# gdoteof/pytorch-zappa-serverless

Hardware: AMD Instinct MI355X
Metric: inferences/sec (whole node) + p50 cold-start ms, ResNet-50 bs=1 at 1/2/4/8 GPU (higher is better)
Workload: dtype bf16

## Files before the change

hipzap/_native.py:

```python
from __future__ import annotations

import ctypes as C
import os
import threading

DEBUG = os.environ.get("HIPZAP_DEBUG") == "1"
_LIB_PATH = os.path.join(os.path.dirname(os.path.realpath(__file__)), "_lib",
                         "libhipzap_debug.so" if DEBUG else "libhipzap.so")
if os.environ.get("HIPZAP_LIB"):
    _LIB_PATH = os.path.realpath(os.environ["HIPZAP_LIB"])
DEBUG_UNITS = ("conv", "gemm", "vision", "transformer", "lstm", "lmbatch", "pack", "block")
_lock = threading.Lock()
_lib = None

c_void_p, c_int, c_long, c_double = C.c_void_p, C.c_int, C.c_long, C.c_double
c_float_p = C.POINTER(C.c_float)

KINDS = {
    "HZ_K_CONV": 1, "HZ_K_LAYERNORM": 2, "HZ_K_EMBED": 3, "HZ_K_ATTENTION": 4, "HZ_K_VIT_TOKENS": 5,
    "HZ_K_LSTM": 6, "HZ_K_DECODER": 7, "HZ_K_SAMPLER": 8, "HZ_K_MAXPOOL": 9, "HZ_K_QUANT": 10,
    "HZ_K_GEMM_FP8": 11, "HZ_K_SOFTMAX": 12, "HZ_K_POOL_FC": 13, "HZ_K_LMB_LAYER": 14, "HZ_K_LMB_DEC": 15,
    "HZ_K_LMB_ADMIT": 16, "HZ_K_STEM": 18, "HZ_K_BNECK": 19, "HZ_K_SEAM": 20, "HZ_K_KCONV": 21,
    "HZ_K_QKVATT": 22, "HZ_K_CONV2": 23, "HZ_K_AVGPOOL": 24, "HZ_K_PREPROCESS": 25, "HZ_K_STEP_BUMP": 26,
    "HZ_K_DIAG": 27, "HZ_K_RESIZE_PREPROCESS": 28,
# ... 196 lines not shown
    _sig(lib, "hz_plan_blob", P, P, C.POINTER(U64))
    _sig(lib, "hz_plan_host", P, P, c_int)
    _sig(lib, "hz_plan_device", P, P, c_int)
    _sig(lib, "hz_plan_stream", P, P, c_int)
    _sig(lib, "hz_plan_upload_stream", P, P)
    _sig(lib, "hz_plan_replay", c_int, P, c_int)
    _sig(lib, "hz_plan_sync", c_int, P, c_int)
    _sig(lib, "hz_plan_infer", c_int, P, c_int, P, U64, U64, P, U64, U64)
    _sig(lib, "hz_plan_bench", D, P, c_int)
    _sig(lib, "hz_plan_close", None, P)
    _sig(lib, "hz_plan_prog", P, P, c_int)
    _sig(lib, "hz_plan_capture_ctx", c_int, P, c_int)
    PP_ = C.POINTER(c_void_p)
    _sig(lib, "hz_exec_create", P, PP_, PP_, PP_, C.POINTER(U64), c_int, PP_, U64, c_int)
    _sig(lib, "hz_exec_create_batched", P, PP_, PP_, PP_, C.POINTER(U64), c_int, PP_, U64, c_int, c_int, D, c_int)
    _sig(lib, "hz_exec_batches", None, P, C.POINTER(U64))
    _sig(lib, "hz_exec_submit", c_int, P, PP_, P, C.POINTER(D))
    _sig(lib, "hz_exec_submit_rows", c_int, P, PP_, c_int, P, C.POINTER(D))
    _sig(lib, "hz_exec_submit_sized", c_int, P, PP_, C.POINTER(U64), P, C.POINTER(D))
    _sig(lib, "hz_exec_stats", None, P, C.POINTER(U64), C.POINTER(U64))
    _sig(lib, "hz_exec_destroy", None, P)
    _sig(lib, "hz_exec_bench", c_int, P, c_int, c_int, PP_, C.POINTER(D), C.POINTER(D))
    _sig(lib, "hz_http_start", P, c_int, P)
    _sig(lib, "hz_http_set_fast", c_int, P, P, c_int, c_int, c_int, c_int, c_int, c_int, C.c_char_p)
    _sig(lib, "hz_http_set_lm", c_int, P, P, c_int, c_int, c_int, c_int, C.c_char_p, U64, C.c_char_p)
    _sig(lib, "hz_http_respond", None, P, c_int, C.c_char_p, U64, C.c_char_p, U64)
    _sig(lib, "hz_http_stats", None, P, C.POINTER(U64))
    _sig(lib, "hz_http_stop", C.c_int, P)
    _sig(lib, "hz_pack_conv_launch", c_int, C.POINTER(PackConvParams), P)
    _sig(lib, "hz_frag_pack_launch", c_int, C.POINTER(FragPackParams), P)
# ... 33 lines not shown
    with _lock:
        if _lib is None:
            if not os.path.exists(_LIB_PATH):
                if os.environ.get("HIPZAP_NO_AUTOBUILD"):
                    raise RuntimeError(f"hipzap native library missing: {_LIB_PATH} (run python -m hipzap.build)")
                from . import build as _b
                _b.build(verbose=False, debug=DEBUG)
            _lib = _load()
    return _lib


def experiments() -> bool:
    return bool(lib().hz_experiments())


def check(rc: int, what: str) -> None:
    if rc != 0:
        raise RuntimeError(f"hipzap native call {what} failed with code {rc}")


def ptr(t) -> int:
    return 0 if t is None else t.data_ptr()


def stream_ptr(stream=None) -> int:
    import torch
    s = stream if stream is not None else torch.cuda.current_stream()
    return s.cuda_stream
```

hipzap/csrc/executor.cpp:

```cpp
#include <hip/hip_runtime.h>

#include <algorithm>
#include <atomic>
#include <chrono>
#include <cstdlib>
#include <condition_variable>
#include <cstring>
#include <deque>
#include <mutex>
#include <thread>
#include <vector>

#include "hipzap.h"

namespace {

constexpr int kMaxIn = 4;

double now_us() {
  return std::chrono::duration<double, std::micro>(std::chrono::steady_clock::now().time_since_epoch()).count();
}

struct Slot {
  HzProgram prog = nullptr;
  hipStream_t st = nullptr;
  void* in[kMaxIn] = {};
  void* out = nullptr;
  hipEvent_t ev = nullptr;
  bool done = false;
  std::atomic<bool> done_a{false};
  int rc = 0;
  std::condition_variable cv;
  int claimed = 0, copied = 0, read = 0;
  bool sealed = false;
  double t_open = 0;
};

struct Exec {
  std::vector<Slot> slots;
  int n_in = 1;
  uint64_t in_bytes[kMaxIn] = {};
  uint64_t out_bytes = 0;
  std::mutex mu;
  std::condition_variable cv_free, cv_work;
  std::vector<int> free_slots;
  std::deque<int> to_launch;
  std::vector<int> inflight;
  bool stop = false;
  int active = 0;
  std::thread worker;
  uint64_t served = 0, polls = 0, batches = 0;
  int rows = 1, open = -1, min_inflight = 1;
  double max_wait_us = 0;
  uint64_t row_in[kMaxIn] = {};
  uint64_t row_out = 0;
  double spin_us = 300.0;
  std::atomic<int> work_hint{0};

  void complete(int s, int rc) {
    std::lock_guard<std::mutex> g(mu);
    slots[s].rc = rc;
    slots[s].done = true;
    slots[s].done_a.store(true, std::memory_order_release);
    slots[s].cv.notify_all();
    served += rows == 1 ? 1 : slots[s].claimed;
    ++batches;
  }

  void queue_if_ready(int s) {
    Slot& sl = slots[s];
    if (sl.sealed && sl.copied == sl.claimed) {
      to_launch.push_back(s);
      work_hint.fetch_add(1, std::memory_order_release);
      cv_work.notify_one();
    }
  }

  void seal_open() {
    const int s = open;
    open = -1;
    slots[s].sealed = true;
    queue_if_ready(s);
  }
// ... 35 lines not shown
      for (size_t i = 0; i < inflight.size();) {
        const int s = inflight[i];
        const hipError_t q = hipEventQuery(slots[s].ev);
        ++polls;
        if (q == hipErrorNotReady) {
          ++i;
          continue;
        }
        complete(s, q == hipSuccess ? 0 : (int)q);
        inflight[i] = inflight.back();
        inflight.pop_back();
        progressed = true;
      }
      if (!progressed) std::this_thread::yield();
    }
  }

  int submit_batched(const void* const* in, void* out, double* lat_us) {
    const double t0 = now_us();
    int s, r;
    {
      std::unique_lock<std::mutex> lk(mu);
      while (open < 0) {
        if (stop) return -10;
        if (!free_slots.empty()) {
          s = free_slots.back();
          free_slots.pop_back();
          Slot& o = slots[s];
          o.claimed = o.copied = o.read = 0;
          o.sealed = o.done = false;
          o.t_open = now_us();
          open = s;
          work_hint.fetch_add(1, std::memory_order_release);
          cv_work.notify_one();
          cv_free.notify_all();
          break;
        }
        cv_free.wait(lk);
      }
      s = open;
      r = slots[s].claimed++;
      if (slots[s].claimed == rows) seal_open();
    }
    Slot& sl = slots[s];
    for (int k = 0; k < n_in; ++k)
      if (in && in[k] && row_in[k]) std::memcpy(static_cast<char*>(sl.in[k]) + r * row_in[k], in[k], row_in[k]);
    int rc;
    {
      std::unique_lock<std::mutex> lk(mu);
      ++sl.copied;
      queue_if_ready(s);
      sl.cv.wait(lk, [&] { return sl.done; });
      rc = sl.rc;
    }
    if (!rc && out && row_out) std::memcpy(out, static_cast<const char*>(sl.out) + r * row_out, row_out);
    {
      std::lock_guard<std::mutex> g(mu);
      if (++sl.read == sl.claimed) {
        free_slots.push_back(s);
        cv_free.notify_all();
      }
// ... 23 lines not shown
            cv_work.notify_one();
            cv_free.notify_all();
            break;
          }
          cv_free.wait(lk);
        }
        s = open;
        r = slots[s].claimed;
        k = std::min(m - done, rows - r);
        slots[s].claimed += k;
        if (slots[s].claimed == rows) seal_open();
      }
      Slot& sl = slots[s];
      for (int q = 0; q < n_in; ++q)
        if (in && in[q] && row_in[q])
          std::memcpy(static_cast<char*>(sl.in[q]) + r * row_in[q], static_cast<const char*>(in[q]) + done * row_in[q],
                      k * row_in[q]);
      {
        std::unique_lock<std::mutex> lk(mu);
        sl.copied += k;
        queue_if_ready(s);
        sl.cv.wait(lk, [&] { return sl.done; });
        rc = sl.rc;
      }
      if (!rc && out && row_out)
        std::memcpy(static_cast<char*>(out) + done * row_out, static_cast<const char*>(sl.out) + r * row_out, k * row_out);
      {
        std::lock_guard<std::mutex> g(mu);
        sl.read += k;
        if (sl.read == sl.claimed) {
          free_slots.push_back(s);
          cv_free.notify_all();
// ... 20 lines not shown
    return rc;
  }

  int submit_one(const void* const* in, void* out, double* lat_us, const uint64_t* nbytes = nullptr) {
    const double t0 = now_us();
    int s;
    {
      std::unique_lock<std::mutex> lk(mu);
      cv_free.wait(lk, [&] { return stop || !free_slots.empty(); });
      if (stop) return -10;
      s = free_slots.back();
      free_slots.pop_back();
    }
    Slot& sl = slots[s];
    for (int k = 0; k < n_in; ++k)
      if (in && in[k] && in_bytes[k]) std::memcpy(sl.in[k], in[k], nbytes ? nbytes[k] : in_bytes[k]);
    int rc;
    bool spin;
    {
      std::unique_lock<std::mutex> lk(mu);
      sl.done = false;
      sl.done_a.store(false, std::memory_order_relaxed);
      to_launch.push_back(s);
      work_hint.fetch_add(1, std::memory_order_release);
      cv_work.notify_one();
      spin = spin_us > 0 && active <= 2;
    }
    if (spin) {
      const double ts = now_us();
      while (!sl.done_a.load(std::memory_order_acquire) && now_us() - ts < 4.0 * spin_us) std::this_thread::yield();
    }
// ... 62 lines not shown
  for (int k = 0; k < n_in; ++k)
    if (in_bytes[k] % rows) return nullptr;
  auto* e = static_cast<Exec*>(hz_exec_create(progs, streams, host_in, in_bytes, n_in, host_out, out_bytes, n));
  if (!e) return nullptr;
  {
    std::lock_guard<std::mutex> g(e->mu);
    e->rows = rows;
    e->max_wait_us = max_wait_us;
    e->min_inflight = min_inflight;
    for (int k = 0; k < n_in; ++k) e->row_in[k] = in_bytes[k] / rows;
    e->row_out = out_bytes / rows;
  }
  return e;
}

void hz_exec_batches(void* h, uint64_t* batches) {
  Exec* e = static_cast<Exec*>(h);
  std::lock_guard<std::mutex> g(e->mu);
  *batches = e->batches;
}

int hz_exec_submit(void* h, const void* const* in, void* out, double* lat_us) {
  return static_cast<Exec*>(h)->submit_wait(in, out, lat_us);
}

int hz_exec_submit_sized(void* h, const void* const* in, const uint64_t* nbytes, void* out, double* lat_us) {
  Exec* e = static_cast<Exec*>(h);
  if (e->rows != 1 || !nbytes) return -1;
  for (int k = 0; k < e->n_in; ++k)
    if (nbytes[k] > e->in_bytes[k]) return -2;
// ... 38 lines not shown
```

hipzap/csrc/hipzap.h:

```cpp
#pragma once
#include <hip/hip_runtime.h>
#include <stdint.h>

#ifdef __cplusplus
extern "C" {
#endif

enum { HZ_ACT_NONE = 0, HZ_ACT_RELU = 1, HZ_ACT_GELU = 2, HZ_ACT_TANH = 3 };

typedef struct HzConvParams {
  const unsigned short* x;
  const unsigned short* w;
  const float* bias;
  const unsigned short* res;
  void* out;
  int N, H, W, C;
  int Cout, R, S, stride, pad, P, Q;
  int M, K, ksteps;
  int act, out_f32, out_rowmajor, ldo;
  int x_rowmajor, ldx;
  int tiles_n;
  int kw;
  const struct HzLnFold* lnf;
  int x_f32;
// ... 458 lines not shown
int hz_prog_add_kernel(HzProgram p, int kind, const void* params, size_t size, int slot);
int hz_prog_add_memcpy(HzProgram p, void* dst, const void* src, size_t bytes, int slot);
int hz_prog_add_fork(HzProgram p, int slot);
int hz_prog_add_join(HzProgram p, int slot);
int hz_prog_run(HzProgram p, hipStream_t st);
int hz_prog_capture(HzProgram p, hipStream_t st);
int hz_prog_replay(HzProgram p, hipStream_t st);
int hz_prog_is_captured(HzProgram p);
int hz_prog_prepare(HzProgram p);
int hz_prog_replay_n(HzProgram p, hipStream_t st, int n);
double hz_prog_bench(HzProgram* progs, hipStream_t* streams, int n, int iters);
int hz_prog_bench2(HzProgram* progs, hipStream_t* streams, int n, int iters, int threads, double* out);
int hz_serve_bench(HzProgram* progs, hipStream_t* streams, void** in_dst, void** in_src, uint64_t in_bytes,
                   void** out_src, void** out_dst, uint64_t out_bytes, int n, int iters, double* lat_us,
                   double* wall_us);
int hz_diag_launch(int kind, int blocks, int threads, void* a, void* b, long bytes, hipStream_t st);

#define HZ_ABI_EPOCH 2
enum { HZ_PLAN_OP_MEMCPY = 6, HZ_PLAN_OP_KERNEL = 7, HZ_PLAN_OP_FORK = 8, HZ_PLAN_OP_JOIN = 9 };
typedef struct HzMemcpyArgs {
  void* dst;
  const void* src;
  uint64_t bytes;
} HzMemcpyArgs;
enum { HZ_PLAN_T_PARSE = 0, HZ_PLAN_T_HIP_INIT = 1, HZ_PLAN_T_UPLOAD = 2, HZ_PLAN_T_CTX_ALLOC = 3,
       HZ_PLAN_T_BIND = 4, HZ_PLAN_T_CAPTURE = 5, HZ_PLAN_T_BLOB_ALLOC = 6,
       HZ_PLAN_T_FIRST_COPY = 7,
       HZ_PLAN_T_STREAM = 8, HZ_PLAN_T_UPLOAD_DMA = 9, HZ_PLAN_T_WARM_WAIT = 10, HZ_PLAN_T_WARM_THREAD = 11,
       HZ_PLAN_NT = 12 };
uint64_t hz_abi_version(void);
// ... 9 lines not shown
void* hz_plan_stream(void* plan, int ctx);
void* hz_plan_upload_stream(void* plan);
int hz_plan_replay(void* plan, int ctx);
int hz_plan_sync(void* plan, int ctx);
int hz_plan_infer(void* plan, int ctx, const void* in, uint64_t in_off, uint64_t in_bytes, void* out,
                  uint64_t out_off, uint64_t out_bytes);
double hz_plan_bench(void* plan, int iters);
HzProgram hz_plan_prog(void* plan, int ctx);
int hz_plan_capture_ctx(void* plan, int ctx);

void* hz_exec_create(HzProgram* progs, hipStream_t* streams, void** host_in, const uint64_t* in_bytes, int n_in,
                     void** host_out, uint64_t out_bytes, int n);
void* hz_exec_create_batched(HzProgram* progs, hipStream_t* streams, void** host_in, const uint64_t* in_bytes,
                             int n_in, void** host_out, uint64_t out_bytes, int n, int rows, double max_wait_us,
                             int min_inflight);
void hz_exec_batches(void* exec, uint64_t* batches);
int hz_exec_submit(void* exec, const void* const* in, void* out, double* lat_us);
int hz_exec_submit_rows(void* exec, const void* const* in, int m, void* out, double* lat_us);
int hz_exec_submit_sized(void* exec, const void* const* in, const uint64_t* nbytes, void* out, double* lat_us);
void hz_exec_stats(void* exec, uint64_t* served, uint64_t* polls);
void hz_exec_destroy(void* exec);
int hz_exec_bench(void* exec, int clients, int iters, const void* const* in, double* lat_us, double* wall_us);

typedef void (*HzHttpPyHandler)(void* req, const char* method, const char* target, const char* headers,
                                uint64_t hlen, const char* body, uint64_t blen);
void* hz_http_start(int listen_fd, HzHttpPyHandler py);
int hz_http_set_fast(void* srv, void* exec, int H, int W, int C, int out_floats, int classes, int probs,
                     const char* model);
int hz_http_set_lm(void* srv, void* sched, int V, int maxn, int dflt, int empty_id, const char* blob, uint64_t blen,
                   const uint8_t* flags);
// ... 9 lines not shown
```

hipzap/csrc/runtime.cpp:

```cpp
#include <hip/hip_runtime.h>
#include <atomic>
#include <chrono>
#include <cstdio>
#include <cstdlib>
#include <cstring>
#include <thread>
#include <vector>

#include "common.h"
#include "hipzap.h"

namespace {

struct Op {
  int slot;
  enum Type { KERNEL, MEMCPY, FORK, JOIN } type;
  int kind;
  std::vector<char> prm;
};

struct Program {
  std::vector<Op> ops;
  std::vector<hipStream_t> side;
  std::vector<hipEvent_t> fork_ev;
  hipGraph_t graph = nullptr;
// ... 199 lines not shown
        if (!rc && out_bytes) memcpy(out_dst[i], out_src[i], out_bytes);
        rcs[i] = rc;
        lat_us[(size_t)i * iters + it] =
            std::chrono::duration<double, std::micro>(std::chrono::steady_clock::now() - a).count();
      }
    });
  for (auto& t : th) t.join();
  *wall_us = std::chrono::duration<double, std::micro>(std::chrono::steady_clock::now() - t0).count();
  int rc = 0;
  for (int r : rcs) rc |= r;
  return rc;
}

}

extern "C" int hz_experiments(void) { return HZ_EXPERIMENTS; }

extern "C" int hz_prog_replay_n(HzProgram h, hipStream_t st, int n) {
  for (int i = 0; i < n; ++i) {
    const int rc = hz_prog_replay(h, st);
    if (rc) return rc;
  }
  return 0;
}

static int hz_conv_op(const HzConvOp* o, hipStream_t st) { return hz_conv_launch(&o->p, o->cfg, st); }
static int hz_conv2_op(const HzConv2Op* o, hipStream_t st) { return hz_conv2_launch(&o->a, &o->b, o->cfg, st); }
static int hz_avgpool_op(const HzAvgpoolArgs* a, hipStream_t st) {
  return hz_avgpool_launch(a->x, a->out, a->N, a->HW, a->C, a->blocked, st);
}
// ... 53 lines not shown
```

hipzap/engine/engine.py:

```python
from __future__ import annotations

import os
import threading
import time

import torch

from .. import _native
from ..models import registry
from .program import ExecContext, bench_contexts, serve_bench_contexts


def load_tuning(model: str, batch: int, contexts: int = 1) -> dict | None:
    import json
    from .tune import table_path
    for c in range(contexts, 0, -1):
        p = table_path(model, batch, c)
        if p.exists():
            with open(p) as f:
                return json.load(f)
    return None


def add_softmax_head(g) -> None:
# ... 153 lines not shown
            return ex
        from ..executor import Executor
        with self._build_lock:
            if getattr(self, "_bexec", None) is not None:
                raise RuntimeError("this engine serves through the dynamic-batching executor")
            if self._exec is None:
                for lk in self._locks:
                    lk.acquire()
                try:
                    cs = self.contexts
                    self._exec = Executor(
                        [c.prog for c in cs], [s.cuda_stream for s in self.streams],
                        [[c.host_inputs[k].data_ptr() for c in cs] for k in range(len(cs[0].host_inputs))],
                        [h.numel() * h.element_size() for h in cs[0].host_inputs],
                        [c.host_output.data_ptr() for c in cs],
                        cs[0].host_output.numel() * cs[0].host_output.element_size())
                finally:
                    for lk in self._locks:
                        lk.release()
        return self._exec

    def infer(self, x) -> torch.Tensor:
        xs = list(x) if isinstance(x, (list, tuple)) else [x]
        ex = self.executor()
        if ex is not None:
            c0 = self.contexts[0]
            hbs = c0.host_inputs
            if all(xi.dtype == hb.dtype and xi.is_contiguous() and xi.numel() == hb.numel() and xi.device.type == "cpu"
                   for hb, xi in zip(hbs, xs)):
                ins = xs
            else:
                ins = [xi.to(hb.dtype).reshape(hb.shape).contiguous() for hb, xi in zip(hbs, xs)]
            out = torch.empty_like(c0.host_output)
            ex.submit([t.data_ptr() for t in ins], out.data_ptr())
            if _native.DEBUG:
                from ..utils import kcheck
                kcheck.check(f"{self.model} infer")
            return self._post(out)
        i = self._pick()
        ctx, s = self.contexts[i], self.streams[i]
        with self._locks[i], torch.cuda.device(self.device), torch.cuda.stream(s):
            if self.host_io:
                for hb, xi in zip(ctx.host_inputs, xs):
                    hb.copy_(xi.reshape(hb.shape))
                ctx.replay(s)
                s.synchronize()
                out = ctx.host_output.clone()
            else:
                for d, xi in zip(ctx.inputs, xs):
                    d.copy_(xi.reshape(d.shape), non_blocking=True)
                ctx.replay(s)
                out = ctx.output.to("cpu", non_blocking=False)
        if _native.DEBUG:
            from ..utils import kcheck
            kcheck.check(f"{self.model} infer")
        return self._post(out)

    @property
    def resize(self) -> dict | None:
# ... 57 lines not shown

    def batched_executor(self, max_wait_us: float = 200.0, min_inflight: int = 1):
        from ..executor import Executor
        self.ensure_contexts()
        with self._build_lock:
            if self._exec is not None:
                raise RuntimeError("this engine already serves through the per-request executor")
            if getattr(self, "_bexec", None) is None:
                cs = self.contexts
                self._bexec = Executor(
                    [c.prog for c in cs], [s.cuda_stream for s in self.streams],
                    [[c.host_inputs[k].data_ptr() for c in cs] for k in range(len(cs[0].host_inputs))],
                    [h.numel() * h.element_size() for h in cs[0].host_inputs],
                    [c.host_output.data_ptr() for c in cs],
                    cs[0].host_output.numel() * cs[0].host_output.element_size(),
                    rows=self.batch, max_wait_us=max_wait_us, min_inflight=min_inflight)
        return self._bexec

    def serve_bench(self, iters: int, payload=None, clients: int | None = None,
                    mode: str = "executor") -> tuple[float, list]:
        self.ensure_contexts()
        c0 = self.contexts[0]
        p = payload if payload is not None else c0.host_input
        p = p.to(c0.host_input.dtype).reshape(c0.host_input.shape).contiguous()
        if mode == "threads":
            return serve_bench_contexts(self.contexts, self.streams, iters, [p.clone() for _ in self.contexts])
        ex = self.executor()
        return ex.bench(clients or len(self.contexts), iters, [p.data_ptr()])

    def describe(self) -> dict:
        c = self.contexts[0]
# ... 81 lines not shown
```

hipzap/engine/fusion.py:

```python
from __future__ import annotations

import ctypes as C
import os
from dataclasses import dataclass

import numpy as np

from .. import _native as N

HZ_K_STEM, HZ_K_BNECK, HZ_K_SEAM, HZ_K_KCONV = N.HZ_K_STEM, N.HZ_K_BNECK, N.HZ_K_SEAM, N.HZ_K_KCONV
KINDS = ("stem", "convpool", "bneck", "bneck2", "seam", "kconv", "tail", "xseam", "dsseam")
DEFAULT = "convpool,bneck,bneck2,seam,kconv,tail,xseam"


@N.params_of("HZ_K_STEM")
class StemParams(C.Structure):
    _fields_ = [("src", C.c_void_p), ("w", C.c_void_p), ("bias", C.c_void_p), ("out", C.c_void_p),
                ("N", C.c_int), ("H", C.c_int), ("W", C.c_int), ("mode", C.c_int),
                ("SH", C.c_int), ("SW", C.c_int), ("PH", C.c_int), ("PW", C.c_int),
                ("norm", C.c_int), ("pad_", C.c_int), ("mean", C.c_float * 4), ("inv_std", C.c_float * 4)]


@N.params_of("HZ_K_BNECK")
class BneckParams(C.Structure):
# ... 34 lines not shown
    next_seam: int | None = None
    reader: int | None = None
    preset: int | None = None
    ds: object | None = None
    ds_from: int | None = None


def enabled_kinds(spec: str | None = None) -> set:
    v = os.environ.get("HIPZAP_FUSE", DEFAULT) if spec is None else spec
    v = v.strip().lower()
    if v in ("", "0", "none", "off"):
        return set()
    if v in ("1", "all", "on"):
        return {"stem", "bneck", "bneck2"}
    return {k for k in v.split(",") if k in KINDS}


def _conv(n, kind="conv"):
    return n is not None and n.kind == kind


def _geom(pc, cin, cout, k, stride, pad) -> bool:
    return (pc.cin == cin and pc.cout == cout and pc.r == k and pc.s == k and pc.stride == stride
            and pc.pad == pad)


def _internal_only(g, grp) -> bool:
    inner = {t for n in grp[:-1] for t in n.outputs}
    if inner & set(g.outputs):
        return False
# ... 523 lines not shown
```

hipzap/engine/plan.py:

```python
from __future__ import annotations

import ctypes as C
import dataclasses
import json
import os
import struct

import torch

from .. import _native as N
from ..lite import PLAN_VERSION
from ..models import registry
from .engine import add_softmax_head, load_tuning
from .program import ExecContext

PLAN_SUFFIX = ".hzplan"
MAGIC = b"HZPLAN01"
VERSION = PLAN_VERSION
HEADER = struct.Struct("<8s15Q")
OPHDR = struct.Struct("<IiiIII")
RELOC = struct.Struct("<IIQ")
OP_MEMCPY, OP_KERNEL, OP_FORK, OP_JOIN = 6, 7, 8, 9
BLOB_ALIGN = 4096
FLAG_WEIGHTLESS = 1
# ... 98 lines not shown

def _dtype_name(dt: torch.dtype) -> str:
    return str(dt).replace("torch.", "")


def export_plan(model: str, params: dict, arch_kw: dict, path: str, batch: int = 1, contexts: int = 1,
                zero_copy: str = "all", probs: bool = False, tuned: dict | None = None,
                source: dict | None = None, host_io: bool = True, weightless: bool = False,
                extra_meta: dict | None = None) -> dict:
    adapter = registry.get(model)
    g = adapter.build_graph(batch=batch, **arch_kw)
    if probs:
        add_softmax_head(g)
    if tuned is None:
        tuned = load_tuning(model, batch, contexts)
    rec = PlanRecorder()
    ctx = ExecContext(g, params, torch.device("cpu"), tuned, host_io=host_io, zero_copy=zero_copy if host_io else "",
                      lib=rec)
    regs = _Regions()
    for key, obj in params.items():
        for field, t in _tensors(obj):
            regs.add(t, 0, True, label=(key, field))
    for t in ctx._keep:
        regs.add(t, 0, True)
    host = (list(ctx.host_inputs) + [ctx.host_output]) if host_io else []
    host_ptrs = {h.untyped_storage().data_ptr() for h in host}
    regs.add(ctx.arena, 1, False)
    for tid, t in ctx.ext.items():
        if t.untyped_storage().data_ptr() not in host_ptrs:
            regs.add(t, 1, False)
# ... 171 lines not shown
```

hipzap/engine/program.py:

```python
from __future__ import annotations

import ctypes as C
import os

import torch

from .. import _native as N
from ..ops import conv as conv_ops
from ..ops import fp8
from ..ops import transformer as tx
from ..ops import vision
from . import fusion
from .graph import Graph, plan_memory


def pair_key(ka: str, kb: str) -> str:
    return f"pair:{ka}|{kb}"


def conv_pairs(g: Graph) -> dict:
    out = {}
    i = 0
    while i + 1 < len(g.nodes):
        a, b = g.nodes[i], g.nodes[i + 1]
# ... 22 lines not shown
            continue
        L, heads, B = att.attrs["L"], att.attrs["heads"], att.attrs["B"]
        pc = params.get(a.get("w"))
        D = heads * 64
        if pc is None or L > 128 or pc.cout != 3 * D or pc.ksteps * 32 != D or pc.bias is None:
            continue
        qkv = gm.outputs[0]
        if qkv in g.outputs or g.shape(qkv) != (B * L, 3 * D) or (a.get("ldx") or g.shape(gm.inputs[0])[-1]) % 8:
            continue
        if any(qkv in n.inputs for j, n in enumerate(nodes) if j != i + 1):
            continue
        if g.tensors[att.outputs[0]].dtype != torch.bfloat16 or g.tensors[gm.inputs[0]].dtype != torch.bfloat16:
            continue
        out[i] = att
    return out


def _ln_folded(n) -> bool:
    a = n.attrs
    return n.kind == "gemm" and bool(a.get("ln_in") or a.get("res_ln") or a.get("stats_out") is not None)


class ExecContext:
    def __init__(self, g: Graph, params: dict, device: torch.device, tuned: dict | None = None,
                 host_io: bool = False, pair_convs: bool | None = None, zero_copy: str | None = None,
                 lib=None, fuse: str | None = None):
        self.graph = g
        self.recording = lib is not None and getattr(lib, "recording", False)
        self.device = torch.device(device)
        self.params = params
        self._keep: list = []
        self._nslab: dict[int, int] = {}
        lib = lib if lib is not None else N.lib()
        self._lib = lib
        self.fused = fusion.plan(g, params, fusion.enabled_kinds(fuse) if fuse is not None else None)
        conv_plans = self._conv_plans(g, params, tuned)
        if pair_convs is None:
            pair_convs = os.environ.get("HIPZAP_PAIR_CONVS", "1") != "0"
        self.pairs = conv_pairs(g) if pair_convs else {}
        paired = set(self.pairs) | set(self.pairs.values())
        self.fused = {k: f for k, f in self.fused.items() if f.kind != "seam" or (
            f.init not in paired and f.consumer not in paired and conv_plans[f.init][0] < 16
            and conv_plans[f.consumer][0] < 16)}
        while True:
            n0 = len(self.fused)
            self.fused = {k: f for k, f in self.fused.items() if f.kind != "kconv" or (
                (f.seam is None or f.seam in self.fused) and (f.next_seam is None or f.next_seam in self.fused)
                and (f.seam is not None or conv_plans[f.preset][0] < 16))}
            self.fused = {k: f for k, f in self.fused.items() if f.kind != "seam" or f.end - f.start == 2 or (
                f.consumer in self.fused and self.fused[f.consumer].kind == "kconv")}
# ... 11 lines not shown
        self.pooled_readers = {id(g.nodes[f.reader]) for f in self.fused.values() if f.kind == "tail"}
        self.kconv_preset = {id(g.nodes[f.preset]): f for f in self.fused.values()
                             if f.kind == "kconv" and f.seam is None}
        self.qkvatt = qkvatt_pairs(g, params)
        offsets, arena_bytes = plan_memory(fusion.planning_graph(g, self.fused),
                                           groups=[(f.start, f.end) for f in self.fused.values()] +
                                           [(i, i + 2) for i in self.qkvatt])
        self.arena_bytes = arena_bytes
        self.arena = torch.empty(max(arena_bytes, 256), dtype=torch.uint8, device=self.device)
        base = self.arena.data_ptr()
        self.ext: dict[int, torch.Tensor] = {}
        for tid, spec in enumerate(g.tensors):
            if spec.external:
                self.ext[tid] = torch.zeros(spec.shape, dtype=spec.dtype, device=self.device)

        def addr(tid):
            if tid is None:
                return 0
            if tid in self.ext:
                return self.ext[tid].data_ptr()
            return base + offsets[tid]

        self._addr = addr
        self.tensor_offsets = offsets
        self.prog = lib.hz_prog_create()
        self.configs: list = []
        self.host_io = host_io
        zc = zero_copy if zero_copy is not None else os.environ.get("HIPZAP_ZERO_COPY", "")
        self.zc_in, self.zc_out = host_io and zc in ("in", "all", "1"), host_io and zc in ("out", "all", "1")
        if host_io:
            pin = (lambda t: t) if self.recording else (lambda t: t.pin_memory())
            self.host_inputs = [pin(torch.zeros(self.ext[t].shape, dtype=self.ext[t].dtype)) for t in g.inputs]
            self.host_input = self.host_inputs[0]
            self.host_output = pin(torch.zeros(self.output.shape, dtype=self.output.dtype))
            for t, hbuf in zip(g.inputs, self.host_inputs):
                if self.zc_in:
                    self.ext[t] = hbuf
                    continue
                d = self.ext[t]
                N.check(lib.hz_prog_add_memcpy(self.prog, d.data_ptr(), hbuf.data_ptr(), d.numel() * d.element_size(),
                                               0), "h2d")
            if self.zc_out:
                self.ext[g.outputs[0]] = self.host_output
        i = 0
        while i < len(g.nodes):
            n = g.nodes[i]
            if i in self.fused:
                f = self.fused[i]
                self.configs.append(fusion.add_fused(self.prog, g, params, f, addr, lib, self.fused))
                i = f.end
                continue
            if i in self.qkvatt:
# ... 276 lines not shown
        elif n.kind == "softmax":
            ishape = g.shape(n.inputs[0])
            rows, ld = ishape[0], int(torch.tensor(ishape[1:]).prod())
            src = g.tensors[n.inputs[0]]
            D = n.attrs.get("D") or ld
            prm = tx.SoftmaxParams(addr(n.inputs[0]), 0, addr(n.outputs[0]), rows, D, ld, g.shape(n.outputs[0])[-1],
                                   int(src.dtype == torch.bfloat16), float(n.attrs.get("scale", 1.0)))
            N.prog_add(lib, self.prog, N.HZ_K_SOFTMAX, prm, n.slot, "add_softmax")
        elif n.kind == "fork":
            N.check(lib.hz_prog_add_fork(self.prog, n.slot), "fork")
        elif n.kind == "join":
            N.check(lib.hz_prog_add_join(self.prog, n.slot), "join")
        else:
            raise NotImplementedError(f"node kind {n.kind}")

    @property
    def input(self) -> torch.Tensor:
        return self.ext[self.graph.inputs[0]]

    @property
    def inputs(self) -> list:
        return [self.ext[t] for t in self.graph.inputs]

    @property
    def output(self) -> torch.Tensor:
        return self.ext[self.graph.outputs[0]]

    def view(self, tid: int) -> torch.Tensor:
        if tid in self.ext:
            return self.ext[tid]
# ... 10 lines not shown
    @property
    def captured(self) -> bool:
        return bool(N.lib().hz_prog_is_captured(self.prog))

    def replay(self, stream=None):
        N.check(N.lib().hz_prog_replay(self.prog, N.stream_ptr(stream)), "prog_replay")

    def num_ops(self) -> int:
        return N.lib().hz_prog_num_ops(self.prog)

    def __del__(self):
        try:
            if getattr(self, "prog", None):
                self._lib.hz_prog_destroy(self.prog)
                self.prog = None
        except Exception:
            pass


def bench_contexts(ctxs: list, streams: list, iters: int, threads: bool | None = None) -> float:
    n = len(ctxs)
    progs = (C.c_void_p * n)(*[c.prog for c in ctxs])
    strs = (C.c_void_p * n)(*[s.cuda_stream for s in streams])
    if threads is None:
        threads = os.environ.get("HIPZAP_SUBMIT_THREADS", "0") == "1"
    if threads and n > 1:
        out = (C.c_double * 2)()
        rc = N.lib().hz_prog_bench2(progs, strs, n, iters, 1, out)
        if rc:
            raise RuntimeError(f"hz_prog_bench2 failed ({rc})")
# ... 26 lines not shown
```

hipzap/executor.py:

```python
from __future__ import annotations

import ctypes as C

from . import _native as N


class Executor:
    def __init__(self, progs: list, streams: list, host_in: list, in_bytes: list, host_out: list, out_bytes: int,
                 rows: int = 1, max_wait_us: float = 200.0, min_inflight: int = 1):
        n, n_in = len(progs), len(in_bytes)
        assert n > 0 and all(len(h) == n for h in host_in) and len(host_out) == n and 0 < n_in <= 4
        V = C.c_void_p
        flat_in = [a for k in range(n_in) for a in host_in[k]]
        self._keep = ((V * n)(*progs), (V * n)(*streams), (V * (n * n_in))(*flat_in),
                      (C.c_uint64 * n_in)(*in_bytes), (V * n)(*host_out))
        self.n, self.n_in, self.rows = n, n_in, rows
        self.out_bytes, self.in_bytes = out_bytes // rows, [b // rows for b in in_bytes]
        if rows > 1:
            h = N.lib().hz_exec_create_batched(self._keep[0], self._keep[1], self._keep[2], self._keep[3], n_in,
                                               self._keep[4], out_bytes, n, rows, float(max_wait_us), min_inflight)
        else:
            h = N.lib().hz_exec_create(self._keep[0], self._keep[1], self._keep[2], self._keep[3], n_in,
                                       self._keep[4], out_bytes, n)
        if not h:
            raise RuntimeError("hz_exec_create failed")
        self._h = h

    def submit(self, in_ptrs: list, out_ptr: int) -> float:
        arr = (C.c_void_p * self.n_in)(*in_ptrs)
        lat = C.c_double()
        rc = N.lib().hz_exec_submit(self._h, arr, out_ptr, C.byref(lat))
        if rc:
            raise RuntimeError(f"executor request failed ({rc})")
        return lat.value * 1e-3

    def submit_sized(self, in_ptrs: list, nbytes: list, out_ptr: int) -> float:
        if self.rows != 1 or len(nbytes) != self.n_in or any(int(b) > cap for b, cap in zip(nbytes, self.in_bytes)):
            raise ValueError(f"submit_sized: {list(nbytes)} bytes for inputs of {self.in_bytes} (rows {self.rows})")
        arr = (C.c_void_p * self.n_in)(*in_ptrs)
        nb = (C.c_uint64 * self.n_in)(*[int(b) for b in nbytes])
        lat = C.c_double()
# ... 43 lines not shown
```

Before: 14300.

## Place request input slots in large-BAR device memory with streaming CPU writes

When zero-copy input is enabled and the device exposes a large BAR, request input buffers are allocated as fine-grained device memory and mapped to a host address obtained via hsa_amd_pointer_info. CPU submitters then write the uint8 image with SSE2 non-temporal stores and an sfence, so the kernels read input from local VRAM instead of over PCIe from pinned host memory. The default fusion set also turns on the stem fusion when device request slots are used. This adds PCIe write traffic on the CPU submit path, depends on HSA internals, and falls back to pinned host memory when the probe fails.

```diff
diff --git a/hipzap/_native.py b/hipzap/_native.py
--- a/hipzap/_native.py
+++ b/hipzap/_native.py
@@ -234,6 +234,12 @@
     PP_ = C.POINTER(c_void_p)
     _sig(lib, "hz_exec_create", P, PP_, PP_, PP_, C.POINTER(U64), c_int, PP_, U64, c_int)
     _sig(lib, "hz_exec_create_batched", P, PP_, PP_, PP_, C.POINTER(U64), c_int, PP_, U64, c_int, c_int, D, c_int)
+    _sig(lib, "hz_exec_set_input_kind", c_int, P, c_int, c_int)
+    _sig(lib, "hz_reqslot_probe", c_int)
+    _sig(lib, "hz_reqslot_alloc", c_int, U64, PP_, PP_, C.POINTER(c_int))
+    _sig(lib, "hz_reqslot_free", c_int, P, c_int)
+    _sig(lib, "hz_reqslot_write", None, P, P, U64, U64)
+    _sig(lib, "hz_reqslot_copy_bench", c_int, PP_, P, U64, c_int, c_int, c_int, C.POINTER(D))
     _sig(lib, "hz_exec_batches", None, P, C.POINTER(U64))
     _sig(lib, "hz_exec_submit", c_int, P, PP_, P, C.POINTER(D))
     _sig(lib, "hz_exec_submit_rows", c_int, P, PP_, c_int, P, C.POINTER(D))
@@ -297,6 +303,20 @@
     return bool(lib().hz_experiments())
 
 
+REQSLOT_PINNED, REQSLOT_DEVICE = 0, 1
+
+
+def reqslot_alloc(nbytes: int):
+    dev, host, kind = c_void_p(), c_void_p(), c_int(0)
+    if lib().hz_reqslot_alloc(int(nbytes), C.byref(dev), C.byref(host), C.byref(kind)) != 0 or not dev.value:
+        return None
+    return dev.value, host.value, kind.value
+
+
+def reqslot_free(dev: int, kind: int) -> None:
+    lib().hz_reqslot_free(dev, kind)
+
+
 def check(rc: int, what: str) -> None:
     if rc != 0:
         raise RuntimeError(f"hipzap native call {what} failed with code {rc}")
diff --git a/hipzap/csrc/executor.cpp b/hipzap/csrc/executor.cpp
--- a/hipzap/csrc/executor.cpp
+++ b/hipzap/csrc/executor.cpp
@@ -12,6 +12,7 @@
 #include <vector>
 
 #include "hipzap.h"
+#include "reqcopy.h"
 
 namespace {
 
@@ -40,6 +41,7 @@
   std::vector<Slot> slots;
   int n_in = 1;
   uint64_t in_bytes[kMaxIn] = {};
+  bool in_dev[kMaxIn] = {};
   uint64_t out_bytes = 0;
   std::mutex mu;
   std::condition_variable cv_free, cv_work;
@@ -67,6 +69,15 @@
     ++batches;
   }
 
+  void put(int k, void* dst, const void* src, uint64_t n, uint64_t cap) const {
+    if (!in_dev[k]) {
+      std::memcpy(dst, src, n);
+      return;
+    }
+    hz_reqcopy(dst, src, (size_t)n, (size_t)cap);
+    hz_reqcopy_fence();
+  }
+
   void queue_if_ready(int s) {
     Slot& sl = slots[s];
     if (sl.sealed && sl.copied == sl.claimed) {
@@ -132,6 +143,11 @@
       }
       if (!progressed) std::this_thread::yield();
     }
+  }
+
+  uint64_t slot_cap(int k) const { return (in_bytes[k] + 15) & ~uint64_t(15); }
+  uint64_t row_cap(int k, int r, int m) const {
+    return r + m == rows ? slot_cap(k) - r * row_in[k] : m * row_in[k];
   }
 
   int submit_batched(const void* const* in, void* out, double* lat_us) {
@@ -162,7 +178,8 @@
     }
     Slot& sl = slots[s];
     for (int k = 0; k < n_in; ++k)
-      if (in && in[k] && row_in[k]) std::memcpy(static_cast<char*>(sl.in[k]) + r * row_in[k], in[k], row_in[k]);
+      if (in && in[k] && row_in[k])
+        put(k, static_cast<char*>(sl.in[k]) + r * row_in[k], in[k], row_in[k], row_cap(k, r, 1));
     int rc;
     {
       std::unique_lock<std::mutex> lk(mu);
@@ -216,8 +233,8 @@
       Slot& sl = slots[s];
       for (int q = 0; q < n_in; ++q)
         if (in && in[q] && row_in[q])
-          std::memcpy(static_cast<char*>(sl.in[q]) + r * row_in[q], static_cast<const char*>(in[q]) + done * row_in[q],
-                      k * row_in[q]);
+          put(q, static_cast<char*>(sl.in[q]) + r * row_in[q], static_cast<const char*>(in[q]) + done * row_in[q],
+              k * row_in[q], row_cap(q, r, k));
       {
         std::unique_lock<std::mutex> lk(mu);
         sl.copied += k;
@@ -268,7 +285,7 @@
     }
     Slot& sl = slots[s];
     for (int k = 0; k < n_in; ++k)
-      if (in && in[k] && in_bytes[k]) std::memcpy(sl.in[k], in[k], nbytes ? nbytes[k] : in_bytes[k]);
+      if (in && in[k] && in_bytes[k]) put(k, sl.in[k], in[k], nbytes ? nbytes[k] : in_bytes[k], nbytes ? nbytes[k] : slot_cap(k));
     int rc;
     bool spin;
     {
@@ -361,6 +378,14 @@
   return e;
 }
 
+int hz_exec_set_input_kind(void* h, int k, int kind) {
+  Exec* e = static_cast<Exec*>(h);
+  if (k < 0 || k >= e->n_in) return -1;
+  std::lock_guard<std::mutex> g(e->mu);
+  e->in_dev[k] = kind == HZ_REQSLOT_DEVICE;
+  return 0;
+}
+
 void hz_exec_batches(void* h, uint64_t* batches) {
   Exec* e = static_cast<Exec*>(h);
   std::lock_guard<std::mutex> g(e->mu);
diff --git a/hipzap/csrc/hipzap.h b/hipzap/csrc/hipzap.h
--- a/hipzap/csrc/hipzap.h
+++ b/hipzap/csrc/hipzap.h
@@ -496,6 +496,13 @@
 int hz_serve_bench(HzProgram* progs, hipStream_t* streams, void** in_dst, void** in_src, uint64_t in_bytes,
                    void** out_src, void** out_dst, uint64_t out_bytes, int n, int iters, double* lat_us,
                    double* wall_us);
+enum { HZ_REQSLOT_PINNED = 0, HZ_REQSLOT_DEVICE = 1 };
+int hz_reqslot_probe(void);
+int hz_reqslot_alloc(uint64_t bytes, void** dev, void** host, int* kind);
+int hz_reqslot_free(void* dev, int kind);
+void hz_reqslot_write(void* dst, const void* src, uint64_t n, uint64_t cap);
+int hz_reqslot_copy_bench(void** slots, const void* src, uint64_t n, int threads, int iters, int streaming,
+                          double* out);
 int hz_diag_launch(int kind, int blocks, int threads, void* a, void* b, long bytes, hipStream_t st);
 
 #define HZ_ABI_EPOCH 2
@@ -535,6 +542,7 @@
 void* hz_exec_create_batched(HzProgram* progs, hipStream_t* streams, void** host_in, const uint64_t* in_bytes,
                              int n_in, void** host_out, uint64_t out_bytes, int n, int rows, double max_wait_us,
                              int min_inflight);
+int hz_exec_set_input_kind(void* exec, int k, int kind);
 void hz_exec_batches(void* exec, uint64_t* batches);
 int hz_exec_submit(void* exec, const void* const* in, void* out, double* lat_us);
 int hz_exec_submit_rows(void* exec, const void* const* in, int m, void* out, double* lat_us);
diff --git a/hipzap/csrc/reqcopy.h b/hipzap/csrc/reqcopy.h
--- /dev/null
+++ b/hipzap/csrc/reqcopy.h
@@ -0,0 +1,69 @@
+#pragma once
+
+#include <cstddef>
+#include <cstdint>
+#include <cstring>
+
+#if defined(__x86_64__) || defined(__i386__)
+#include <emmintrin.h>
+#define HZ_REQCOPY_SSE2 1
+#else
+#include <atomic>
+#define HZ_REQCOPY_SSE2 0
+#endif
+
+static inline void hz_reqcopy(void* dst, const void* src, size_t n, size_t cap) {
+  unsigned char* d = static_cast<unsigned char*>(dst);
+  const unsigned char* s = static_cast<const unsigned char*>(src);
+  auto small = [&](size_t m) {
+    for (size_t w = 8; w; w >>= 1)
+      if (m & w) {
+        std::memcpy(d, s, w);
+        d += w, s += w;
+      }
+  };
+  const size_t mis = reinterpret_cast<uintptr_t>(d) & 15;
+  if (mis) {
+    const size_t head = 16 - mis < n ? 16 - mis : n;
+    small(head);
+    n -= head;
+    cap -= head;
+  }
+#if HZ_REQCOPY_SSE2
+  size_t i = 0;
+  for (; i + 64 <= n; i += 64) {
+    const __m128i a = _mm_loadu_si128(reinterpret_cast<const __m128i*>(s + i));
+    const __m128i b = _mm_loadu_si128(reinterpret_cast<const __m128i*>(s + i + 16));
+    const __m128i c = _mm_loadu_si128(reinterpret_cast<const __m128i*>(s + i + 32));
+    const __m128i e = _mm_loadu_si128(reinterpret_cast<const __m128i*>(s + i + 48));
+    _mm_stream_si128(reinterpret_cast<__m128i*>(d + i), a);
+    _mm_stream_si128(reinterpret_cast<__m128i*>(d + i + 16), b);
+    _mm_stream_si128(reinterpret_cast<__m128i*>(d + i + 32), c);
+    _mm_stream_si128(reinterpret_cast<__m128i*>(d + i + 48), e);
+  }
+  for (; i + 16 <= n; i += 16)
+    _mm_stream_si128(reinterpret_cast<__m128i*>(d + i), _mm_loadu_si128(reinterpret_cast<const __m128i*>(s + i)));
+  d += i, s += i;
+  n -= i, cap -= i;
+  if (n) {
+    if (cap >= 16) {
+      alignas(16) unsigned char last[16] = {};
+      std::memcpy(last, s, n);
+      _mm_stream_si128(reinterpret_cast<__m128i*>(d), _mm_load_si128(reinterpret_cast<const __m128i*>(last)));
+    } else {
+      small(n);
+    }
+  }
+#else
+  (void)cap;
+  std::memcpy(d, s, n);
+#endif
+}
+
+static inline void hz_reqcopy_fence() {
+#if HZ_REQCOPY_SSE2
+  _mm_sfence();
+#else
+  std::atomic_thread_fence(std::memory_order_seq_cst);
+#endif
+}
diff --git a/hipzap/csrc/runtime.cpp b/hipzap/csrc/runtime.cpp
--- a/hipzap/csrc/runtime.cpp
+++ b/hipzap/csrc/runtime.cpp
@@ -1,4 +1,8 @@
 #include <hip/hip_runtime.h>
+#include <hsa/hsa.h>
+#include <hsa/hsa_ext_amd.h>
+#include <dlfcn.h>
+#include <algorithm>
 #include <atomic>
 #include <chrono>
 #include <cstdio>
@@ -9,6 +13,7 @@
 
 #include "common.h"
 #include "hipzap.h"
+#include "reqcopy.h"
 
 namespace {
 
@@ -238,6 +243,113 @@
 
 }
 
+namespace {
+
+using PointerInfoFn = hsa_status_t (*)(const void*, hsa_amd_pointer_info_t*, void* (*)(size_t), uint32_t*,
+                                       hsa_agent_t**);
+
+void* reported_host_address(void* dev) {
+  static const PointerInfoFn fn = reinterpret_cast<PointerInfoFn>(dlsym(RTLD_DEFAULT, "hsa_amd_pointer_info"));
+  if (!fn || !dev) return nullptr;
+  hsa_amd_pointer_info_t pi;
+  memset(&pi, 0, sizeof(pi));
+  pi.size = sizeof(pi);
+  if (fn(dev, &pi, nullptr, nullptr, nullptr) != HSA_STATUS_SUCCESS) return nullptr;
+  if (pi.type != HSA_EXT_POINTER_TYPE_HSA || !pi.hostBaseAddress || !pi.agentBaseAddress) return nullptr;
+  const char* base = static_cast<const char*>(pi.agentBaseAddress);
+  const char* p = static_cast<const char*>(dev);
+  if (p < base || p >= base + pi.sizeInBytes) return nullptr;
+  return static_cast<char*>(pi.hostBaseAddress) + (p - base);
+}
+
+bool reqslot_disabled() {
+  const char* e = getenv("HIPZAP_REQSLOT");
+  return e && (!strcmp(e, "host") || !strcmp(e, "0") || !strcmp(e, "off"));
+}
+
+}
+
+extern "C" int hz_reqslot_probe(void) {
+  static std::atomic<int> cache[64];
+  if (reqslot_disabled()) return 0;
+  int d = -1, large_bar = 0;
+  if (hipGetDevice(&d) != hipSuccess || d < 0 || d >= 64) return 0;
+  if (const int c = cache[d].load()) return c - 1;
+  int yes = 0;
+  if (hipDeviceGetAttribute(&large_bar, hipDeviceAttributeIsLargeBar, d) == hipSuccess && large_bar) {
+    void* p = nullptr;
+    if (hipExtMallocWithFlags(&p, 4096, hipDeviceMallocFinegrained) == hipSuccess) {
+      yes = reported_host_address(p) != nullptr;
+      (void)hipFree(p);
+    }
+  }
+  (void)hipGetLastError();
+  cache[d].store(yes + 1);
+  return yes;
+}
+
+extern "C" int hz_reqslot_alloc(uint64_t bytes, void** dev, void** host, int* kind) {
+  if (!dev || !host || !kind) return -1;
+  *dev = *host = nullptr;
+  *kind = HZ_REQSLOT_PINNED;
+  const size_t cap = bytes ? (size_t(bytes) + 15) & ~size_t(15) : 256;
+  if (hz_reqslot_probe()) {
+    void* p = nullptr;
+    if (hipExtMallocWithFlags(&p, cap, hipDeviceMallocFinegrained) == hipSuccess) {
+      void* h = reported_host_address(p);
+      if (h && hipMemset(p, 0, cap) == hipSuccess && hipDeviceSynchronize() == hipSuccess) {
+        *dev = p;
+        *host = h;
+        *kind = HZ_REQSLOT_DEVICE;
+        return 0;
+      }
+      (void)hipFree(p);
+    }
+    (void)hipGetLastError();
+  }
+  void* p = nullptr;
+  const hipError_t e = hipHostMalloc(&p, cap, hipHostMallocDefault);
+  if (e != hipSuccess) return (int)e;
+  memset(p, 0, cap);
+  *dev = *host = p;
+  return 0;
+}
+
+extern "C" int hz_reqslot_free(void* dev, int kind) {
+  if (!dev) return 0;
+  return (int)(kind == HZ_REQSLOT_DEVICE ? hipFree(dev) : hipHostFree(dev));
+}
+
+extern "C" void hz_reqslot_write(void* dst, const void* src, uint64_t n, uint64_t cap) {
+  hz_reqcopy(dst, src, (size_t)n, (size_t)cap);
+  hz_reqcopy_fence();
+}
+
+extern "C" int hz_reqslot_copy_bench(void** slots, const void* src, uint64_t n, int threads, int iters,
+                                     int streaming, double* out) {
+  if (threads < 1 || iters < 1 || !slots || !src || !out) return -1;
+  std::vector<std::vector<double>> v(threads);
+  std::vector<std::thread> th;
+  for (int t = 0; t < threads; ++t)
+    th.emplace_back([&, t] {
+      for (int it = 0; it < iters; ++it) {
+        const auto a = std::chrono::steady_clock::now();
+        if (streaming)
+          hz_reqslot_write(slots[t], src, n, (n + 15) & ~uint64_t(15));
+        else
+          memcpy(slots[t], src, n);
+        v[t].push_back(std::chrono::duration<double, std::micro>(std::chrono::steady_clock::now() - a).count());
+      }
+    });
+  for (auto& t : th) t.join();
+  std::vector<double> all;
+  for (auto& x : v) all.insert(all.end(), x.begin(), x.end());
+  std::sort(all.begin(), all.end());
+  out[0] = all.front();
+  out[1] = all[all.size() / 2];
+  return 0;
+}
+
 extern "C" int hz_experiments(void) { return HZ_EXPERIMENTS; }
 
 extern "C" int hz_prog_replay_n(HzProgram h, hipStream_t st, int n) {
diff --git a/hipzap/engine/engine.py b/hipzap/engine/engine.py
--- a/hipzap/engine/engine.py
+++ b/hipzap/engine/engine.py
@@ -191,7 +191,8 @@
                         [[c.host_inputs[k].data_ptr() for c in cs] for k in range(len(cs[0].host_inputs))],
                         [h.numel() * h.element_size() for h in cs[0].host_inputs],
                         [c.host_output.data_ptr() for c in cs],
-                        cs[0].host_output.numel() * cs[0].host_output.element_size())
+                        cs[0].host_output.numel() * cs[0].host_output.element_size(),
+                        in_kinds=[cs[0].input_kind] * len(cs[0].host_inputs))
                 finally:
                     for lk in self._locks:
                         lk.release()
@@ -218,8 +219,8 @@
         ctx, s = self.contexts[i], self.streams[i]
         with self._locks[i], torch.cuda.device(self.device), torch.cuda.stream(s):
             if self.host_io:
-                for hb, xi in zip(ctx.host_inputs, xs):
-                    hb.copy_(xi.reshape(hb.shape))
+                for k, xi in enumerate(xs[:len(ctx.host_inputs)]):
+                    ctx.write_input(k, xi)
                 ctx.replay(s)
                 s.synchronize()
                 out = ctx.host_output.clone()
@@ -307,7 +308,8 @@
                     [h.numel() * h.element_size() for h in cs[0].host_inputs],
                     [c.host_output.data_ptr() for c in cs],
                     cs[0].host_output.numel() * cs[0].host_output.element_size(),
-                    rows=self.batch, max_wait_us=max_wait_us, min_inflight=min_inflight)
+                    rows=self.batch, max_wait_us=max_wait_us, min_inflight=min_inflight,
+                    in_kinds=[cs[0].input_kind] * len(cs[0].host_inputs))
         return self._bexec
 
     def serve_bench(self, iters: int, payload=None, clients: int | None = None,
diff --git a/hipzap/engine/fusion.py b/hipzap/engine/fusion.py
--- a/hipzap/engine/fusion.py
+++ b/hipzap/engine/fusion.py
@@ -72,6 +72,12 @@
     if v in ("1", "all", "on"):
         return {"stem", "bneck", "bneck2"}
     return {k for k in v.split(",") if k in KINDS}
+
+
+def default_kinds(device_u8_request: bool) -> set:
+    if "HIPZAP_FUSE" in os.environ or not device_u8_request:
+        return enabled_kinds()
+    return enabled_kinds(DEFAULT) | {"stem"}
 
 
 def _conv(n, kind="conv"):
diff --git a/hipzap/engine/plan.py b/hipzap/engine/plan.py
--- a/hipzap/engine/plan.py
+++ b/hipzap/engine/plan.py
@@ -136,6 +136,9 @@
         add_softmax_head(g)
     if tuned is None:
         tuned = load_tuning(model, batch, contexts)
+    if zero_copy == "dev":
+        raise ValueError("plan images keep their request slots in the context's pinned host block: "
+                         "zero_copy='dev' (device-resident request slots) is an Engine option")
     rec = PlanRecorder()
     ctx = ExecContext(g, params, torch.device("cpu"), tuned, host_io=host_io, zero_copy=zero_copy if host_io else "",
                       lib=rec)
diff --git a/hipzap/engine/program.py b/hipzap/engine/program.py
--- a/hipzap/engine/program.py
+++ b/hipzap/engine/program.py
@@ -60,6 +60,15 @@
             continue
         out[i] = att
     return out
+
+
+REQSLOT_DEFAULT = "dev"
+
+
+def _slot_view(slot, like: torch.Tensor) -> torch.Tensor:
+    _, host, _, nbytes = slot
+    raw = torch.frombuffer((C.c_uint8 * nbytes).from_address(host), dtype=torch.uint8)
+    return raw.view(like.dtype).reshape(like.shape)
 
 
 def _ln_folded(n) -> bool:
@@ -79,7 +88,15 @@
         self._nslab: dict[int, int] = {}
         lib = lib if lib is not None else N.lib()
         self._lib = lib
-        self.fused = fusion.plan(g, params, fusion.enabled_kinds(fuse) if fuse is not None else None)
+        self.host_io = host_io
+        zc = zero_copy if zero_copy is not None else os.environ.get("HIPZAP_ZERO_COPY", "")
+        self._req_slots = self._request_slots(g, params, zc, fuse) if host_io else None
+        self.input_kind = N.REQSLOT_DEVICE if self._req_slots else N.REQSLOT_PINNED
+        zc = "all" if zc == "dev" else zc
+        u8_request = len(g.inputs) == 1 and g.tensors[g.inputs[0]].dtype == torch.uint8
+        kinds = fusion.enabled_kinds(fuse) if fuse is not None else \
+            fusion.default_kinds(self.input_kind == N.REQSLOT_DEVICE and u8_request)
+        self.fused = fusion.plan(g, params, kinds)
         conv_plans = self._conv_plans(g, params, tuned)
         if pair_convs is None:
             pair_convs = os.environ.get("HIPZAP_PAIR_CONVS", "1") != "0"
@@ -121,9 +138,13 @@
             if spec.external:
                 self.ext[tid] = torch.zeros(spec.shape, dtype=spec.dtype, device=self.device)
 
+        self._dev_addr: dict[int, int] = {}
+
         def addr(tid):
             if tid is None:
                 return 0
+            if tid in self._dev_addr:
+                return self._dev_addr[tid]
             if tid in self.ext:
                 return self.ext[tid].data_ptr()
             return base + offsets[tid]
@@ -132,17 +153,20 @@
         self.tensor_offsets = offsets
         self.prog = lib.hz_prog_create()
         self.configs: list = []
-        self.host_io = host_io
-        zc = zero_copy if zero_copy is not None else os.environ.get("HIPZAP_ZERO_COPY", "")
         self.zc_in, self.zc_out = host_io and zc in ("in", "all", "1"), host_io and zc in ("out", "all", "1")
         if host_io:
             pin = (lambda t: t) if self.recording else (lambda t: t.pin_memory())
-            self.host_inputs = [pin(torch.zeros(self.ext[t].shape, dtype=self.ext[t].dtype)) for t in g.inputs]
+            if self._req_slots:
+                self.host_inputs = [_slot_view(s, self.ext[t]) for s, t in zip(self._req_slots, g.inputs)]
+            else:
+                self.host_inputs = [pin(torch.zeros(self.ext[t].shape, dtype=self.ext[t].dtype)) for t in g.inputs]
             self.host_input = self.host_inputs[0]
             self.host_output = pin(torch.zeros(self.output.shape, dtype=self.output.dtype))
-            for t, hbuf in zip(g.inputs, self.host_inputs):
+            for k, (t, hbuf) in enumerate(zip(g.inputs, self.host_inputs)):
                 if self.zc_in:
                     self.ext[t] = hbuf
+                    if self._req_slots:
+                        self._dev_addr[t] = self._req_slots[k][0]
                     continue
                 d = self.ext[t]
                 N.check(lib.hz_prog_add_memcpy(self.prog, d.data_ptr(), hbuf.data_ptr(), d.numel() * d.element_size(),
@@ -449,6 +473,36 @@
         else:
             raise NotImplementedError(f"node kind {n.kind}")
 
+    def _request_slots(self, g, params, zc: str, fuse) -> list | None:
+        if zc != "dev":
+            if zc not in ("all", "1") or self.recording or fuse is not None or \
+                    os.environ.get("HIPZAP_REQSLOT", REQSLOT_DEFAULT) != "dev":
+                return None
+            if len(g.inputs) != 1 or g.tensors[g.inputs[0]].dtype != torch.uint8 or \
+                    not any(fusion.match_stem(g, params, i) for i in range(len(g.nodes))):
+                return None
+        slots = []
+        self._slot_free = N.reqslot_free
+        for t in g.inputs:
+            spec = g.tensors[t]
+            s = N.reqslot_alloc(spec.nbytes)
+            if s is not None:
+                slots.append((*s, spec.nbytes))
+            if s is None or s[2] != N.REQSLOT_DEVICE:
+                for dev, _, kind, _ in slots:
+                    N.reqslot_free(dev, kind)
+                return None
+        return slots
+
+    def write_input(self, k: int, x: torch.Tensor) -> None:
+        hb = self.host_inputs[k]
+        if not self._req_slots:
+            hb.copy_(x.reshape(hb.shape))
+            return
+        src = x.detach().to("cpu", hb.dtype).reshape(hb.shape).contiguous()
+        _, host, _, nbytes = self._req_slots[k]
+        N.lib().hz_reqslot_write(host, src.data_ptr(), nbytes, (nbytes + 15) // 16 * 16)
+
     @property
     def input(self) -> torch.Tensor:
         return self.ext[self.graph.inputs[0]]
@@ -489,6 +543,9 @@
             if getattr(self, "prog", None):
                 self._lib.hz_prog_destroy(self.prog)
                 self.prog = None
+            for dev, _, kind, _ in getattr(self, "_req_slots", None) or []:
+                self._slot_free(dev, kind)
+            self._req_slots = None
         except Exception:
             pass
 
diff --git a/hipzap/executor.py b/hipzap/executor.py
--- a/hipzap/executor.py
+++ b/hipzap/executor.py
@@ -7,7 +7,7 @@
 
 class Executor:
     def __init__(self, progs: list, streams: list, host_in: list, in_bytes: list, host_out: list, out_bytes: int,
-                 rows: int = 1, max_wait_us: float = 200.0, min_inflight: int = 1):
+                 rows: int = 1, max_wait_us: float = 200.0, min_inflight: int = 1, in_kinds: list | None = None):
         n, n_in = len(progs), len(in_bytes)
         assert n > 0 and all(len(h) == n for h in host_in) and len(host_out) == n and 0 < n_in <= 4
         V = C.c_void_p
@@ -25,6 +25,8 @@
         if not h:
             raise RuntimeError("hz_exec_create failed")
         self._h = h
+        for k, kind in enumerate(in_kinds or []):
+            N.check(N.lib().hz_exec_set_input_kind(h, k, int(kind)), "exec_set_input_kind")
 
     def submit(self, in_ptrs: list, out_ptr: int) -> float:
         arr = (C.c_void_p * self.n_in)(*in_ptrs)
```

After: 15120, median of 6. 1.06x the previous value.
